# hartikainen/mujoco_mpc

Measured on AMD Instinct MI355X. Metric: candidate rollouts/s (horizon x samples), higher is better.
Workload: dtype f64

## Files before the change

### mujoco_mpc_amd/csrc/host.h

```cpp
#pragma once
#include <stdlib.h>
#include <stdint.h>
#include <string.h>
#include <map>
#include <mutex>
#include <string>
#include <vector>
#include "../../include/mjpc_hip.h"
#include "model.h"

struct PackedModel {
  std::vector<int> ib;
  std::vector<double> db;
  DevModel M;
  Lay L;
  size_t task_i0, task_d0, task_i_cap, task_d_cap;
  size_t cache_i, cache_d;
  size_t hot_i = 0, hot_d = 0;
  int slab_doubles = 0;
  std::string error;
};

namespace mjpc_host {

// ... 87 lines not shown
        case TBL_CONST:
          if (ty < 1 || id < 0 || id > t->num_dbl - ty) return fail(trm + ": constants dbl_data[" + std::to_string(id) + " .. +" + std::to_string(ty) + ") out of range (num_dbl = " + std::to_string(t->num_dbl) + ")");
          len = ty; break;
        case TBL_PARAM: len = t->num_parameter; break;
        case TBL_QPOS: len = M.nq; break;
        case TBL_QVEL: len = M.nv; break;
        case TBL_ACT: if (M.na == 0) return fail(trm + ": ACT on a model without activation states (na = 0)"); len = M.na; break;
        case TBL_CTRL: case TBL_ACTUATOR_FORCE: len = M.nu; break;
        case TBL_KEY_QPOS: if (!obj(M.nkey, "key")) return false; len = M.nq; break;
        case TBL_MOCAP_POS: case TBL_MOCAP_QUAT: case TBL_MOCAP_MAT:
          if (!obj(M.nmocap, "mocap body")) return false;
          len = kind == TBL_MOCAP_POS ? 3 : (kind == TBL_MOCAP_QUAT ? 4 : 9); break;
        case TBL_SUBTREE_COM: case TBL_SUBTREE_LINVEL: if (!obj(M.nbody, "body")) return false; len = 3; break;
        case TBL_POS: case TBL_QUAT: case TBL_MAT: case TBL_XAXIS: case TBL_YAXIS: case TBL_ZAXIS: case TBL_LINVEL: case TBL_ANGVEL:
          if (ty == MJPC_OBJ_BODY || ty == MJPC_OBJ_XBODY) { if (!obj(M.nbody, "body")) return false; }
          else if (ty == MJPC_OBJ_GEOM) { if (!obj(M.ngeom, "geom")) return false; }
          else if (ty == MJPC_OBJ_SITE) { if (!obj(M.nsite, "site")) return false; }
          else return fail(trm + ": unknown object type " + std::to_string(ty));
          len = kind == TBL_QUAT ? 4 : (kind == TBL_MAT ? 9 : 3); break;
        default: return fail(trm + ": unknown source kind " + std::to_string(kind));
      }
      if (op == TBL_OP_SUBQUAT && ((kind != TBL_QUAT && kind != TBL_MOCAP_QUAT) || off != 0)) return fail(trm + ": SUBQUAT takes two quaternion sources (QUAT / MOCAP_QUAT) at offset 0");
      if (off < 0 || off > len - ncomp) return fail(trm + ": components [" + std::to_string(off) + ", " + std::to_string(off) + " + " + std::to_string(ncomp) + ") beyond the source's length " + std::to_string(len));
    }
    row += dim; term += n;
  }
  if (row != t->num_residual) return fail("the blocks end at row " + std::to_string(row) + ", num_residual is " + std::to_string(t->num_residual));
  if (term != nt) return fail("the blocks use " + std::to_string(term) + " of the " + std::to_string(nt) + " terms");
  return true;
}

static inline void make_layout(const PackedModel &p, Lay &L, const MjpcHipModel *m, const MjpcHipTask *t, int P_max, size_t cache_d, size_t cache_i, bool lean = false, bool reg_solver = false, unsigned spill = 0, int *slab_doubles = nullptr, int *scratch = nullptr) {
  const DevModel &M = p.M;
  int nb = m->nbody, nj = m->njnt, nv = m->nv, ng = m->ngeom, ns = m->nsite, nu = m->nu;
  int o = 0, so = 0;
  int nvp = M.nvp, ne = M.nefcmax, nc = M.nconmax, nr = t->num_residual;
#define A_(f, n) L.f = o; o += (int)(n)
#define S_(bit, f, n) if (spill & (bit)) { L.f = LAY_SLAB(so); so += (int)(n); } else { A_(f, n); }
  A_(qpos, m->nq); A_(qvel, nv); A_(ctrl, nu + 1 + 2 * m->na);
  A_(qacc, nv); A_(qacc_ws, nv); A_(qacc_smooth, nv); A_(qfrc_smooth, nv);
  A_(qfrc_bias, nv); A_(qfrc_constraint, nv); A_(actuator_force, nu + 1); A_(mocap_pos, 3 * m->nmocap + 3); A_(mocap_quat, 4 * m->nmocap + 4);
  A_(xpos, 3 * nb); A_(xquat, 4 * nb); A_(xmat, 9 * nb); A_(xipos, 3 * nb); A_(ximat, 9 * nb); A_(xanchor, 3 * nj + 3); A_(xaxis, 3 * nj + 3);
  A_(geom_xpos, 3 * ng + 3); A_(geom_xmat, 9 * ng + 9); A_(site_xpos, 3 * ns + 3);
#define B_(f, n) if (!lean) { A_(f, n); }
  A_(subtree_com, 3 * nb); B_(cinert, 10 * nb); B_(crb, 10 * nb); A_(cdof, 6 * nv + 18); A_(cvel, 6 * nb); B_(cdof_dot, 6 * nv + 18);
  B_(cacc, 6 * nb); B_(cfrc, 6 * nb); B_(cfrc_sub, 6 * nb); A_(subtree_linvel, 3 * nb); A_(bodytmp, 3 * nb);
#undef B_
  A_(qM, nv * nvp + 1); A_(qL, nv * nvp + 1);
  A_(qH, (lean && reg_solver && nv > 32) ? 1 : nv * nvp + 1);
  A_(Linv, nv + 1); A_(Hinv, nv + 1);
  int ja_rows = ((ne - M.nfric + 7) & ~7) + (m->cone == MJPC_CONE_ELLIPTIC ? ((nc + 3) & ~3) : 0) + 4 + ((M.ntfric + 3) & ~3);
  
  S_(SPILL_EFC_J, efc_J, (ne - M.nfric) * nvp + 1);
  int ja_need = 64 + ne * 7 + nc * 17 + (m->cone == MJPC_CONE_ELLIPTIC ? (nc * nv + 7) / 8 + (nc * nv + 3) / 4 + (MJPC_SIDE_JOB > 0 ? 3 : 2) * nv * nvp : 0);
  int ja_size = reg_solver ? ja_need + 1 : ja_rows * nvp + 1;
  if (ja_size < ja_need) ja_size = ja_need;
  S_(SPILL_EFC_JA, efc_JA, ja_size);
  if (scratch) *scratch = ((spill & SPILL_EFC_J) != 0) == ((spill & SPILL_EFC_JA) != 0) ? (ne - M.nfric) * nvp + 1 + ja_size : (ne - M.nfric) * nvp + 1;
  if (lean) {
    int q = L.efc_JA;
    L.cinert = q; q += 10 * nb; L.crb = q; q += 10 * nb; L.cdof_dot = q; q += 6 * nv + 18;
    L.cacc = q; q += 6 * nb; L.cfrc = q; q += 6 * nb; L.cfrc_sub = q; q += 6 * nb;
    if (q > o) o = q;
  }
  S_(SPILL_EFC_VEC, efc_D, ne); S_(SPILL_EFC_VEC, efc_R, ne); S_(SPILL_EFC_VEC, efc_aref, ne); S_(SPILL_EFC_VEC, efc_force, ne);
  S_(SPILL_EFC_VEC, efc_jar, ne); S_(SPILL_EFC_VEC, efc_jv, ne); S_(SPILL_EFC_VEC, efc_floss, ne); S_(SPILL_EFC_VEC, efc_pos, ne);
  L.efc_margin = L.efc_jv; L.efc_diag = L.efc_force;
  S_(SPILL_CONTACT, contact, nc * M.con_stride + 1);
  A_(Ma, nv + 1); A_(grad, nv + 1); A_(Mgrad, nv + 1); A_(search, nv + 1); A_(Mv, nv + 1); A_(vtmp, nv + 1); A_(sgl, 4 * nv + 1);
  if (lean) { L.knot_times = 0; L.knot_values = 0; } else { A_(knot_times, P_max); A_(knot_values, P_max * nu + 1); }
  A_(residual, nr + 1); A_(terms, t->num_term + 1); A_(red, 8); A_(prof, 26);
  A_(scr_a, nv + 1); A_(scr_b, nv + 1);
  if (lean) L.xfrc = 0; else { A_(xfrc, 6 * nb); }
  if (m->noslip_iterations > 0) { S_(SPILL_NOSLIP, noslip, ne * nvp + nc * 36 + 2 * ne + 1); } else L.noslip = 0;
  A_(mc_d, cache_d + 1); A_(mc_i, (cache_i + 2) / 2);
  L.ints = o;
#undef S_
#undef A_
  if (slab_doubles) *slab_doubles = so ? so + nvp + 64 : 0;
  int io = 0;
  L.i_efc_type = io; io += ne; L.i_efc_id = io; io += ne; L.i_efc_state = io; io += ne; L.i_efc_dof = io; io += ne;
  L.i_con = io; io += nc * CONI_STRIDE; L.i_active = io; io += (ne + nc + M.ntfric > MAX_ACTIVE_PAIRS ? ne + nc + M.ntfric : MAX_ACTIVE_PAIRS); L.i_misc = io; io += MISC_INTS;
  L.i_hpair = io; if (!lean) io += M.nhpair + nv;
  L.total_doubles = o + (io + 1) / 2;
}

static inline bool build(PackedModel &p, const MjpcHipModel *m, const MjpcHipTask *t, int P_max, bool use_cache = true, bool lean = false, bool hot_only = false, bool reg_solver = false, int spill_mode = SPILL_NONE) {
  p.ib.clear(); p.db.clear(); p.error.clear(); p.slab_doubles = 0;
  DevModel &M = p.M;
  memset(&M, 0, sizeof(M));
  int nb = m->nbody, nj = m->njnt, nv = m->nv, ng = m->ngeom, ns = m->nsite, nu = m->nu;
  if (nv > 64) { p.error = "nv > 64 not supported (dof bitmask)"; return false; }
  {
    int cnt = 0;
    for (int i = 0; i < nu && m->actuator_dyntype; i++) if (m->actuator_dyntype[i] != MJPC_DYN_NONE) {
      int dt = m->actuator_dyntype[i], a = m->actuator_actadr ? m->actuator_actadr[i] : -1;
      if (dt < 0 || dt > MJPC_DYN_FILTEREXACT) { p.error = "actuator " + std::to_string(i) + ": dyntype " + std::to_string(dt) + " not supported (integrator / filter / filterexact only)"; return false; }
      if (a < 0 || a >= m->na || !m->actuator_dynprm || !m->actuator_actlimited || !m->actuator_actrange) { p.error = "actuator " + std::to_string(i) + ": activation address outside [0, na) or missing actuator_dynprm / actlimited / actrange"; return false; }
      cnt++;
    }
    if (cnt != m->na) { p.error = "na = " + std::to_string(m->na) + " but " + std::to_string(cnt) + " stateful actuators (one activation each)"; return false; } }
  if (m->solver != MJPC_SOL_NEWTON) { p.error = "only the Newton solver (mjSOL_NEWTON) is implemented"; return false; }
  if (m->integrator != MJPC_INT_EULER && m->integrator != MJPC_INT_IMPLICITFAST && m->integrator != MJPC_INT_IMPLICIT) { p.error = "only the Euler (with implicit joint damping), implicitfast and implicit integrators are implemented (not RK4)"; return false; }
  if (m->noslip_iterations < 0) { p.error = "noslip_iterations < 0"; return false; }
  for (int e = 0; e < m->neq; e++) {
    if (!m->eq_type || !m->eq_obj1id || !m->eq_obj2id || !m->eq_active0 || !m->eq_data || !m->eq_solref || !m->eq_solimp) { p.error = "neq > 0 but the eq_* tables are missing"; return false; }
    if (!m->eq_active0[e]) continue;
// ... 466 lines not shown
```

### mujoco_mpc_amd/csrc/linalg.h

```cpp
#pragma once
#include <type_traits>
#include "dmath.h"
#include "model.h"

struct Ctx;

#ifndef MJPC_EMU
DEV double readlane_d(double v, int lane) {
  int lo = __builtin_amdgcn_readlane(__double2loint(v), lane);
  int hi = __builtin_amdgcn_readlane(__double2hiint(v), lane);
  return __hiloint2double(hi, lo);
}
#endif

DEV void chol_factor_lds(double *A, double *Linv, double *tmp, int n, int nvp) {
  for (int j = 0; j < n; j++) {
    SYNC();
    PFOR(ii, n - j) {
      int i = j + ii;
      double s = A[i * nvp + j];
#pragma unroll 4
      for (int k = 0; k < j; k++) s -= A[i * nvp + k] * A[j * nvp + k];
      tmp[i] = s;
    }
    SYNC();
    double t = tmp[j];
    if (t < D_MINVAL) t = D_MINVAL;
    double dj = sqrt(t), inv = 1.0 / dj;
    PFOR(ii, n - j) {
      int i = j + ii;
      A[i * nvp + j] = (i == j) ? dj : tmp[i] * inv;
    }
    if (LANE == 0) Linv[j] = inv;
  }
  SYNC();
}
DEV void chol_solve_lds(const double *L, const double *Linv, double *x, int n, int nvp) {
  for (int i = 0; i < n; i++) {
    SYNC();
    double xi = x[i] * Linv[i];
    SYNC();
    PFOR(kk, n - i - 1) { int k = i + 1 + kk; x[k] -= L[k * nvp + i] * xi; }
    if (LANE == 0) x[i] = xi;
  }
  for (int i = n - 1; i >= 0; i--) {
    SYNC();
    double xi = x[i] * Linv[i];
    SYNC();
    PFOR(k, i) x[k] -= L[i * nvp + k] * xi;
    if (LANE == 0) x[i] = xi;
  }
  SYNC();
}

#ifndef MJPC_EMU
template <int N>
struct LDLRegs { double lo[N], up[N], rinv; };
struct LDLExtra { const double *x[3]; int n; const double *row; };

template <int I, int E, class F>
DEV void static_for(F &&f) {
  if constexpr (I < E) { f(std::integral_constant<int, I>{}); static_for<I + 1, E>(f); }
}
template <int N>
DEV void ldl_load_row(const double *A, int nvp, const LDLExtra *ex, double *a, double &dg) {
  const int i = LANE;
  const bool act = i < N;
  if (ex && ex->row) {
    double d0 = 1.0;
    static_for<0, N>([&](auto jc) { constexpr int j = decltype(jc)::value; a[j] = act ? ex->row[j] : 0.0; d0 = (j == i) ? ex->row[j] : d0; });
    dg = act ? d0 : 1.0;
  } else {
    static_for<0, N>([&](auto jc) { constexpr int j = decltype(jc)::value; a[j] = act ? A[(j <= i) ? i * nvp + j : j * nvp + i] : 0.0; });
    dg = act ? A[i * nvp + i] : 1.0;
  }
  if (ex && ex->n > 0) {
    const int nx = ex->n;
    double t[3][N], td[3];
#pragma unroll
    for (int w = 0; w < 3; w++) {
      const double *X = ex->x[w < nx ? w : 0];
      static_for<0, N>([&](auto jc) { constexpr int j = decltype(jc)::value; t[w][j] = X[(j <= i && act) ? i * nvp + j : (act ? j * nvp + i : 0)]; });
      td[w] = X[act ? i * nvp + i : 0];
      if (w + 1 >= nx) break;
    }
    __builtin_amdgcn_sched_barrier(0);
#pragma unroll
    for (int w = 0; w < 3; w++) {
      if (w >= nx) break;
      static_for<0, N>([&](auto jc) { constexpr int j = decltype(jc)::value; a[j] += act ? t[w][j] : 0.0; });
      dg += act ? td[w] : 0.0;
    }
  }
}
template <int N>
DEV void ldl_factor_regs(const double *A, int nvp, LDLRegs<N> &f, const LDLExtra *ex = nullptr) {
  static_assert(N >= 1 && N <= 64, "one matrix row per lane");
  const int i = LANE;
  const bool act = i < N;
  double a[N];
  double dg;
  ldl_load_row<N>(A, nvp, ex, a, dg);
  static_for<1, N>([&](auto kc) {
    constexpr int k = N - decltype(kc)::value;
    double rk = readlane_d(fast_rcp(dg < D_MINVAL ? D_MINVAL : dg), k);
    double hk = a[k];
    double l = (i < k) ? hk * rk : 0.0;
    dg -= l * hk;
    static_for<0, (k + 7) / 8>([&](auto gc) {
      constexpr int j0 = decltype(gc)::value * 8;
      double sj[8];
      static_for<0, 8>([&](auto qc) { constexpr int q = decltype(qc)::value; if constexpr (j0 + q < k) sj[q] = readlane_d(a[j0 + q], k); });
      __builtin_amdgcn_sched_barrier(0);
      static_for<0, 8>([&](auto qc) { constexpr int q = decltype(qc)::value; if constexpr (j0 + q < k) a[j0 + q] -= l * sj[q]; });
      __builtin_amdgcn_sched_barrier(0);
    });
    f.up[k] = l;
  });
  f.up[0] = 0.0;
  if (dg < D_MINVAL) dg = D_MINVAL;
  f.rinv = fast_rcp(dg);
  static_for<0, N>([&](auto jc) { constexpr int j = decltype(jc)::value; f.lo[j] = (act && j < i) ? a[j] * f.rinv : 0.0; });
}
template <int N>
DEV double ldl_solve_regs(const LDLRegs<N> &f, double xi) {
  static_for<1, N>([&](auto kc) { constexpr int k = N - decltype(kc)::value; xi -= f.up[k] * readlane_d(xi, k); });
  xi *= f.rinv;
  static_for<0, N - 1>([&](auto jc) { constexpr int j = decltype(jc)::value; xi -= f.lo[j] * readlane_d(xi, j); });
  return xi;
}
template <int N> constexpr int tree_depth(int k) { int d = 0; for (int a = DofTree<N>::parent(k); a >= 0; a = DofTree<N>::parent(a)) d++; return d; }
template <int N> constexpr int tree_nth_anc(int k, int n) { int a = DofTree<N>::parent(k); for (int q = 0; q < n; q++) a = DofTree<N>::parent(a); return a; }
template <int N> constexpr int tree_height(int k) {
  int h = 0;
  for (int c = k + 1; c < N; c++) if (DofTree<N>::parent(c) == k) { int hc = tree_height<N>(c) + 1; if (hc > h) h = hc; }
  return h;
}
template <int N> constexpr int tree_nlevel() { int h = 0; for (int k = 0; k < N; k++) { int hk = tree_height<N>(k); if (hk > h) h = hk; } return h + 1; }
template <int N> constexpr int tree_level_npair(int H) { int n = 0; for (int k = N - 1; k >= 1; k--) if (tree_height<N>(k) == H) n += tree_depth<N>(k); return n; }
template <int N> constexpr int tree_level_pair(int H, int e, bool pivot) {
  for (int k = N - 1; k >= 1; k--) if (tree_height<N>(k) == H) {
    int d = tree_depth<N>(k);
    if (e < d) return pivot ? k : tree_nth_anc<N>(k, e);
    e -= d;
  }
// ... 150 lines not shown
```

### mujoco_mpc_amd/csrc/model.h

```cpp
#pragma once
#include <stdint.h>

#define CON_STRIDE_ELLIPTIC 45
#define NVP_OF(n) ((((n) + 1)) | 1)
#define CON_STRIDE_PLAIN 27
#define CON_DIST 0
#define CON_POS 1
#define CON_FRAME 4
#define CON_INCLUDEMARGIN 13
#define CON_FRICTION 14
#define CON_SOLREF 19
#define CON_SOLIMP 21
#define CON_MU 26
#define CON_H 27
#ifndef MJPC_SIDE_JOB
#define MJPC_SIDE_JOB 0
#endif
#define CONI_STRIDE 4
#define MAX_ACTIVE_PAIRS 192
#define EFC_CON_ID(ci, dim, r0) ((ci) | ((dim) << 8) | ((r0) << 16))
#define EFC_CON_CI(id) ((id) & 255)
#define EFC_CON_DIM(id) (((id) >> 8) & 255)
#define EFC_CON_R0(id) ((id) >> 16)

template <int N> struct DofTree { static constexpr bool known = false; static constexpr int parent(int) { return -1; } static constexpr int real_parent(int) { return -1; } };
template <> struct DofTree<18> {
  static constexpr bool known = true;
  static constexpr int parent(int k) { constexpr int p[18] = {-1, 0, 1, 2, 3, 4, 5, 6, 7, 5, 9, 10, 5, 12, 13, 5, 15, 16}; return p[k]; }
  static constexpr int real_parent(int k) { return parent(k); }
};
template <> struct DofTree<27> {
  static constexpr bool known = true;
  static constexpr int parent(int k) {
    constexpr int p[27] = {-1, 0, 1, 2, 3, 4, 5, 6, 7, 8, 9, 10, 11, 12, 13, 8, 15, 16, 17, 18, 19, 5, 21, 22, 5, 24, 25};
    return p[k];
  }
  static constexpr int real_parent(int k) { return parent(k); }
};
template <> struct DofTree<33> {
  static constexpr bool known = true;
  static constexpr int parent(int k) {
    constexpr int p[33] = {-1, 0, 1, -1, 3, 4, 5, 6, 7,  8, 9, 10, 11, 12, 13, 10, 15, 16, 17, 10, 19, 20, 21, 10, 23, 24, 25, 26, 10, 28, 29, 30, 31};
    return p[k];
  }
  static constexpr int real_parent(int k) { return k == 9 ? -1 : parent(k); }
};
template <int N> constexpr bool dof_tree_matches(const int *dof_parentid) {
  if (!DofTree<N>::known) return false;
  for (int k = 0; k < N; k++) if (dof_parentid[k] != DofTree<N>::real_parent(k)) return false;
  return true;
}
static inline int pattern_parent(int nv, int tree_ok, const int *dof_parentid, int k) {
  if (!tree_ok) return dof_parentid[k];
  if (nv == 18) return DofTree<18>::parent(k);
  if (nv == 27) return DofTree<27>::parent(k);
  if (nv == 33) return DofTree<33>::parent(k);
  return dof_parentid[k];
// ... 137 lines not shown
```

### mujoco_mpc_amd/csrc/solver_reg.h

```cpp
#pragma once
#ifndef MJPC_EMU
#ifndef LS_PREDICT
#define LS_PREDICT 1
#endif

template <int NVT> struct HLay {
  static constexpr int G0 = 64 / NVT;
  static constexpr int G = G0 < 1 ? 1 : (G0 > NVT ? NVT : G0);
  static constexpr int CB = (NVT + G - 1) / G;
};
DEV int readlane_i(int v, int lane) { return __builtin_amdgcn_readlane(v, lane); }
#define LSR_STRIDE 7
#define LSC_STRIDE 17
#define LS_ROWREC(c) ((c).efc_JA + 64)
#define LS_CONREC(c) ((c).efc_JA + 64 + (c).M->nefcmax * LSR_STRIDE)

template <int NVT>
DEV void hblock_add_rows(const Ctx &c, double *h, unsigned long long mask, int rbase, double wlane, int hi, int j0) {
  constexpr int nvp = NVP_OF(NVT), CB = HLay<NVT>::CB;
  while (mask) {
    int b0 = (int)__builtin_ctzll(mask); mask &= mask - 1;
    int b1 = b0; double sel1 = 0.0;
    if (mask) { b1 = (int)__builtin_ctzll(mask); mask &= mask - 1; sel1 = 1.0; }
    double w0 = readlane_d(wlane, b0), w1 = readlane_d(wlane, b1) * sel1;
// ... 30 lines not shown
  const int nefc = c.nefc, ns = c.nsingle;
  for (int base = 0; base < nefc; base += NLANE) {
    int r = base + LANE, rc = r < nefc ? r : nefc - 1;
    int st = c.efc_state[rc], type = c.efc_type[rc];
    double D = c.efc_D[rc];
    int flag = r < nefc && r >= ns && st == STATE_QUADRATIC;
    (void)type;
    unsigned long long mask = __builtin_amdgcn_ballot_w64(flag != 0);
    hblock_add_rows<NVT>(c, hq, mask, base, D, hi, j0);
  }
}

template <int NVT>
DEV void newton_grad_reg(Ctx &c, int hi, int hg, bool hact) {
  constexpr int nvp = NVP_OF(NVT), G = HLay<NVT>::G;
  const int ns = c.nsingle, n = c.nefc - ns;
  double part = 0;
  const int trips = (n + G - 1) / G;
  for (int t0 = 0; t0 < trips; t0 += 8) {
    double f[8], j[8];
#pragma unroll
    for (int u = 0; u < 8; u++) {
      int rr = (t0 + u) * G + hg;
      int r = ns + (rr < n ? rr : 0);
      f[u] = c.efc_force[r]; j[u] = c.efc_J[r * nvp + hi];
    }
    __builtin_amdgcn_sched_barrier(0);
#pragma unroll
    for (int u = 0; u < 8; u++) { int rr = (t0 + u) * G + hg; double pr = j[u] * f[u]; part += (rr < n) ? pr : 0.0; }
    __builtin_amdgcn_sched_barrier(0);
  }
  double *sc = c.efc_JA;
  if (hact) sc[hg * NVT + hi] = part;
  SYNC();
  if (LANE < NVT) {
    int i = LANE;
    double jtf = 0;
#pragma unroll
    for (int g = 0; g < G; g++) jtf += sc[g * NVT + i];
    double gr = c.Ma[i] - c.qfrc_smooth[i] - (c.sgl[i] + c.sgl[2 * NVT + i]) - jtf;
    c.grad[i] = gr;
    c.Mgrad[i] = gr;
  }
  SYNC();
}

#define HX_JOBW 18
#define HX_SIDEFROM 21
#define HX_NITEMS 45
#define HX_WDONE HX_HDONE
#define JOBW(seq, np, kind) (((seq) << 4) | ((np) << 2) | (kind))
#define MJPC_NW (MJPC_NH + 1)
#define CONE_BASE(c) ((c).efc_JA + 64 + (c).M->nefcmax * LSR_STRIDE + (c).M->nconmax * LSC_STRIDE)
#define CONE_DOFS(c) ((unsigned char *)CONE_BASE(c))
#define CONE_ITEMS(c) ((unsigned short *)(CONE_BASE(c) + ((c).M->nconmax * NVT + 7) / 8))
#define CONE_PARTIAL(c, w) (CONE_BASE(c) + ((c).M->nconmax * NVT + 7) / 8 + ((c).M->nconmax * NVT + 3) / 4 + (w) * (NVT * NVP_OF(NVT)))

template <int NVT, int DIMT>
DEV void cone_rows(const Ctx &c, double *part, int p0, int pstep) {
  constexpr int nvp = NVP_OF(NVT);
  const int nitems = uniform_i(c.misc[HX_NITEMS]), stride = c.M->con_stride;
  const unsigned short *items = CONE_ITEMS(c);
  const double *crec = LS_CONREC(c);
  for (int it0 = p0 * NLANE; it0 < nitems; it0 += pstep * NLANE) {
    const int it = it0 + LANE;
    const bool valid = it < nitems;
    const int item = items[valid ? it : 0];
    const int ci = item & 255, a = item >> 8;
    const int info = ((const int *)(crec + ci * LSC_STRIDE + 14))[0];
    const int r0 = info >> 16, dim = (info >> 8) & 255;
    const unsigned char *dofs = CONE_DOFS(c) + ci * NVT;
    const int i = dofs[a];
    const int st = c.efc_state[r0];
    const double *cf = c.contact + ci * stride + CON_H;
    double P[DIMT], Q[DIMT], T[DIMT], ji[DIMT];
#pragma unroll
    for (int k = 0; k < DIMT; k++) { P[k] = cf[k]; Q[k] = cf[6 + k]; T[k] = cf[12 + k]; }
    const double *Jr = c.efc_J + r0 * nvp;
#pragma unroll
    for (int k = 0; k < DIMT; k++) ji[k] = Jr[(DIMT <= 3 || k < dim ? k : 0) * nvp + i];
    __builtin_amdgcn_sched_barrier(0);
    const bool active = valid && st == STATE_CONE;
#if defined(MJPC_PROFILE) && !defined(MJPC_EMU)
    if (MJPC_PROFILE_WAVE != 0 && WAVE_ID() == MJPC_PROFILE_WAVE) { int na_ = __builtin_popcountll(__builtin_amdgcn_ballot_w64(active)); if (LANE == 0) { c.prof[23] += na_; c.prof[22] += (it0 == p0 * NLANE); } }
#endif
    if constexpr (DIMT > 3) {
#pragma unroll
      for (int k = 3; k < DIMT; k++) { const bool in = k < dim; P[k] = in ? P[k] : 0.0; Q[k] = in ? Q[k] : 0.0; T[k] = in ? T[k] : 0.0; ji[k] = in ? ji[k] : 0.0; }
    }
    double pi = P[0] * ji[0], qi = Q[1] * ji[1];
#pragma unroll
    for (int k = 1; k < DIMT; k++) { pi += P[k] * ji[k]; if (k > 1) qi += Q[k] * ji[k]; }
    double t[DIMT];
    t[0] = P[0] * pi + Q[0] * ji[0];
#pragma unroll
    for (int k = 1; k < DIMT; k++) t[k] = P[k] * pi - Q[k] * qi + (T[k] * T[k]) * ji[k];
    double *prow = part + i * nvp;
    PROFW(c, 16);
    for (int b = 0; __builtin_amdgcn_ballot_w64(active && b <= a) != 0; b += 2) {
      const bool on0 = active && b <= a, on1 = active && b + 1 <= a;
      const int j0 = dofs[on0 ? b : 0], j1 = dofs[on1 ? b + 1 : 0];
      double x0[DIMT], x1[DIMT];
#pragma unroll
      for (int k = 0; k < DIMT; k++) { x0[k] = Jr[(DIMT <= 3 || k < dim ? k : 0) * nvp + j0]; x1[k] = Jr[(DIMT <= 3 || k < dim ? k : 0) * nvp + j1]; }
      __builtin_amdgcn_sched_barrier(0);
      double v0 = t[0] * x0[0], v1 = t[0] * x1[0];
#pragma unroll
      for (int k = 1; k < DIMT; k++) { v0 += t[k] * x0[k]; v1 += t[k] * x1[k]; }
      if (on0) __builtin_amdgcn_ds_atomic_fadd_f64((__attribute__((address_space(3))) double *)(prow + j0), v0);
      if (on1) __builtin_amdgcn_ds_atomic_fadd_f64((__attribute__((address_space(3))) double *)(prow + j1), v1);
    }
  }
}

#if MJPC_HELPER
DEV int jobw_load(const Ctx &c) { return __builtin_amdgcn_readfirstlane(__hip_atomic_load(c.misc + HX_JOBW, __ATOMIC_RELAXED, __HIP_MEMORY_SCOPE_WORKGROUP)); }
template <int NVT>
DEV int job_post(Ctx &c, int kind, int &side_in) {
  if (c.M->cone != 1) return 0;
  const int seq = ++c.hseq;
  if (MJPC_SIDE_JOB > 0 && !side_in && (seq & 255) >= MJPC_SIDE_JOB) {
    const int base = seq & ~255;
    int ok = 0;
    for (int n = 0; n < (1 << 21); n++) {
      int from = __builtin_amdgcn_readfirstlane(__hip_atomic_load(c.misc + HX_SIDEFROM, __ATOMIC_RELAXED, __HIP_MEMORY_SCOPE_WORKGROUP));
      if (from > base) { ok = 1; break; }
    }
    if (!ok) c.warning |= WARN_SYNC;
    side_in = 1;
  }
  const int np = MJPC_NH + (side_in ? 1 : 0);
  flag_set(c.misc + HX_JOBW, JOBW(seq, np, kind));
  return np;
}
DEV void job_wait(Ctx &c, int np) {
  const int seq = c.hseq;
  for (int k = 0; k < np; k++) if (!flag_wait(c.misc + HX_WDONE + k, seq)) c.warning |= WARN_SYNC;
}
template <int NVT, int DIMT>
DEV void worker_job(Ctx &c, int W, int np, int seq) {
  constexpr int nvp = NVP_OF(NVT);
  PROFW(c, 12);
  double *part = CONE_PARTIAL(c, W);
  PFOR(e, NVT * nvp) part[e] = 0;
  PROFW(c, 15);
  cone_rows<NVT, DIMT>(c, part, W, np);
  PROFW(c, 13);
  flag_set(c.misc + HX_WDONE + W, seq);
  PROFW(c, 14);
}
template <int NVT, int DIMT>
DEV void worker_loop_d(Ctx &c, int W, int last) {
  if (W != 0 && c.nefc > 0 && !flag_wait(c.misc + HX_LSREC, (last >> 8) + 1)) return;
  for (;;) {
    int word = 0, ok = 0;
    for (int n = 0; n < (1 << 21); n++) { word = jobw_load(c); if ((word >> 4) > last) { ok = 1; break; } }
    __builtin_amdgcn_fence(__ATOMIC_ACQUIRE, "workgroup");
    if (!ok) return;
    const int kind = word & 3, np = (word >> 2) & 3;
    if (kind == 0) return;
    last = word >> 4;
    if (W < np) worker_job<NVT, DIMT>(c, W, np, last);
  }
}
template <int NVT>
DEV void worker_loop(Ctx &c, int W, int last) {
  if (c.M->cone != 1) return;
  if (c.M->maxdim <= 3) worker_loop_d<NVT, 3>(c, W, last); else worker_loop_d<NVT, 6>(c, W, last);
}
template <int NVT>
DEV void side_worker(Ctx &c, int t) {
  if (c.M->cone != 1 || MJPC_SIDE_JOB <= 0) return;
  const int base = t * 256;
  int word = jobw_load(c);
  int last = base;
  if ((word >> 4) > base) {
    if ((word & 3) == 0) return;
    last = word >> 4;
  }
  if (LANE == 0) __hip_atomic_store(c.misc + HX_SIDEFROM, last + 1, __ATOMIC_RELAXED, __HIP_MEMORY_SCOPE_WORKGROUP);
  worker_loop<NVT>(c, MJPC_NH, last);
}
#endif

template <int NVT, int DIMT>
DEV void newton_assemble(Ctx &c, const double *hq, int hi, int hg, int j0, bool hact) {
  constexpr int nvp = NVP_OF(NVT), CB = HLay<NVT>::CB;
  double a[CB];
  const double dg = c.sgl[NVT + hi] + c.sgl[3 * NVT + hi];
#pragma unroll
  for (int q = 0; q < CB; q++) a[q] = hq[q] + ((j0 + q == hi) ? dg : 0.0);
#if !MJPC_HELPER
  if (c.M->cone == 1) {
    double *part = CONE_PARTIAL(c, 0);
    PFOR(e, NVT * nvp) part[e] = 0;
    cone_rows<NVT, DIMT>(c, part, 0, 1);
    SYNC();
#pragma unroll
    for (int q = 0; q < CB; q++) a[q] += (hact && j0 + q <= hi) ? part[hi * nvp + j0 + q] : 0.0;
  }
#endif
  if (hact) {
#pragma unroll
    for (int q = 0; q < CB; q++) if (j0 + q < NVT) c.qH[hi * nvp + j0 + q] = a[q];
  }
  SYNC();
}
template <int NVT>
DEV void newton_direction_np(Ctx &c, int np) {
  if (np > 0) {
    LDLExtra ex;
    ex.row = nullptr;
    ex.n = np;
#pragma unroll
    for (int w = 0; w < 3; w++) ex.x[w] = CONE_PARTIAL(c, w < np ? w : 0);
    newton_direction_sum<NVT>(c, ex);
  } else newton_direction<NVT>(c);
}

template <int NVT>
DEV void newton_direction_rows(Ctx &c, const double *hq, int hi, bool hact, int np) {
  if constexpr (HLay<NVT>::G != 1) return;
  double row[NVT];
  const double dg = c.sgl[NVT + hi] + c.sgl[3 * NVT + hi];
#pragma unroll
  for (int q = 0; q < NVT; q++) row[q] = hact ? hq[q] + ((q == hi) ? dg : 0.0) : 0.0;
  LDLExtra ex;
  ex.row = row;
  ex.n = np;
#pragma unroll
  for (int w = 0; w < 3; w++) ex.x[w] = CONE_PARTIAL(c, w < np ? w : 0);
  chol_factor_solve_reg<NVT>(c.qH, c.Mgrad, NVP_OF(NVT), c.M->tree_ok && !c.cross, &ex);
  PROF(c, 17);
}

template <int DIMT>
struct LSReg {
  double lo[LS_RPL], hi[LS_RPL], hD[LS_RPL], F[LS_RPL], X[LS_RPL], V[LS_RPL], DV[LS_RPL], DVV[LS_RPL], rJ[LS_RPL];
  int rinfo[LS_RPL];
  double N0[LS_CPL], NV[LS_CPL], t0[LS_CPL], t1[LS_CPL], t2[LS_CPL], c0[LS_CPL], c1[LS_CPL], c2[LS_CPL], mu[LS_CPL], Dm[LS_CPL];
  int on[LS_CPL], cdim[LS_CPL], crow[LS_CPL], cwasq[LS_CPL];
  int nslot, ncslot;
};

template <int NVT>
DEV void ls_records_build(Ctx &c) {
  constexpr int nvp = NVP_OF(NVT);
  const int nefc = c.nefc, ncon = c.ncon, ns = c.nsingle, nfr = c.M->nfric;
  double *rrec = LS_ROWREC(c), *crec = LS_CONREC(c);
  PFOR(r, nefc) {
    int type = c.efc_type[r], dof = c.efc_dof[r];
    double D = c.efc_D[r], f = c.efc_floss[r], Rf = c.efc_R[r] * f;
    int single = r < ns;
    double rj = single ? (r < nfr ? 1.0 : c.efc_J[r * nvp + dof]) : 0.0;
    int quad = type != CNSTR_CONTACT_ELLIPTIC;
    int fric = quad && type <= CNSTR_FRICTION_TENDON;
    double *o = rrec + r * LSR_STRIDE;
    o[0] = fric ? -Rf : (quad ? -1e300 : -1.0); o[1] = fric ? Rf : (quad ? 0.0 : 1.0);
    o[2] = quad ? 0.5 * D : 0.0; o[3] = fric ? f : 0.0; o[4] = rj;
    ((int *)(o + 5))[0] = quad | (fric << 1) | ((quad && single) << 2) | ((single ? dof : 0) << 8);
    o[6] = D;
  }
  int nc_lane = 0;
  PFOR(ci, ncon) {
    int dim = c.con_i[ci * CONI_STRIDE], i = c.con_i[ci * CONI_STRIDE + 3];
    const double *cc = c.contact + ci * c.M->con_stride;
    int on = dim > 1 && c.efc_type[i] == CNSTR_CONTACT_ELLIPTIC;
    double mu = cc[CON_MU];
    double *o = crec + ci * LSC_STRIDE;
    for (int j = 0; j < 6; j++) {
      int use = on && j < dim;
      double fr = j == 0 ? mu : cc[CON_FRICTION + j - 1];
      double Dj = c.efc_D[use ? i + j : i];
      o[j] = use ? Dj * fast_rcp(fr * fr) : 0.0;
      o[6 + j] = use ? fr : 0.0;
    }
    o[12] = on ? mu : 0.0;
    o[13] = on ? c.efc_D[i] * fast_rcp(mu * mu * (1 + mu * mu)) : 0.0;
    ((int *)(o + 14))[0] = on | (dim << 8) | (i << 16);
    int nc = 0;
    if (on) {
      unsigned long long m = MDM()[MI(geom_bodyid)[c.con_i[ci * CONI_STRIDE + 1]]] | MDM()[MI(geom_bodyid)[c.con_i[ci * CONI_STRIDE + 2]]];
      unsigned char *dl = CONE_DOFS(c) + ci * NVT;
      while (m) { int dd = (int)__builtin_ctzll(m); m &= m - 1; dl[nc++] = (unsigned char)dd; }
    }
    ((int *)(o + 14))[2] = nc;
    nc_lane = nc;
  }
  {
    int total, off = wave_excl_scan(nc_lane, &total);
    unsigned short *il = CONE_ITEMS(c) + off;
    for (int a = 0; a < nc_lane; a++) il[a] = (unsigned short)(LANE | (a << 8));
    if (LANE == 0) c.misc[HX_NITEMS] = total;
  }
  SYNC();
}

template <int NVT, int DIMT>
DEV void ls_load_reg(Ctx &c, LSReg<DIMT> &d) {
  const int nefc = c.nefc, ncon = c.ncon, last = c.nefc - 1;
  const double *rrec = LS_ROWREC(c), *crec = LS_CONREC(c);
  d.nslot = (nefc + NLANE - 1) / NLANE; d.ncslot = (ncon + NLANE - 1) / NLANE;
#pragma unroll
  for (int k = 0; k < LS_RPL; k++) {
    d.lo[k] = -1; d.hi[k] = 1; d.hD[k] = 0; d.F[k] = 0; d.X[k] = 0; d.V[k] = 0; d.DV[k] = 0; d.DVV[k] = 0; d.rJ[k] = 0; d.rinfo[k] = 0;
    if (k < d.nslot) {
      int r = LANE + NLANE * k, rc = r < nefc ? r : last;
      const double *o = rrec + rc * LSR_STRIDE;
      double lo = o[0], hi = o[1], hD = o[2], F = o[3], rj = o[4];
      int info = ((const int *)(o + 5))[0], st = c.efc_state[rc];
      double v = c.efc_jv[rc], x = c.efc_jar[rc];
      __builtin_amdgcn_sched_barrier(0);
      const bool ok = r < nefc;
      d.X[k] = ok ? x : 0.0; d.V[k] = ok ? v : 0.0;
      d.lo[k] = ok ? lo : -1.0; d.hi[k] = ok ? hi : 1.0; d.hD[k] = ok ? hD : 0.0; d.F[k] = ok ? F : 0.0; d.rJ[k] = rj;
      d.rinfo[k] = ok ? (info | ((st == STATE_QUADRATIC) << 3)) : 0;
      double dv = 2 * d.hD[k] * d.V[k];
      d.DV[k] = dv; d.DVV[k] = dv * d.V[k];
    }
  }
#pragma unroll
  for (int q = 0; q < LS_CPL; q++) {
    d.on[q] = 0; d.mu[q] = 0; d.Dm[q] = 0; d.cdim[q] = 0; d.crow[q] = 0; d.cwasq[q] = 0;
    d.N0[q] = 0; d.NV[q] = 0; d.t0[q] = 0; d.t1[q] = 0; d.t2[q] = 0; d.c0[q] = 0; d.c1[q] = 0; d.c2[q] = 0;
    if (q < d.ncslot) {
      int ci = LANE + NLANE * q, cic = ci < ncon ? ci : ncon - 1;
      const double *o = crec + cic * LSC_STRIDE;
      int info = ((const int *)(o + 14))[0];
      double E[DIMT], fr[DIMT];
#pragma unroll
      for (int j = 0; j < DIMT; j++) { E[j] = o[j]; fr[j] = o[6 + j]; }
      double mu = o[12], Dm = o[13];
      int on = (ci < ncon) && (info & 1), dim = (info >> 8) & 255, i = info >> 16;
      double jv[DIMT], jr[DIMT];
#pragma unroll
      for (int j = 0; j < DIMT; j++) { int rj = i + j < nefc ? i + j : last; jv[j] = c.efc_jv[rj]; jr[j] = c.efc_jar[rj]; }
      int st0 = c.efc_state[i];
      __builtin_amdgcn_sched_barrier(0);
      d.on[q] = on; d.mu[q] = on ? mu : 0.0; d.Dm[q] = on ? Dm : 0.0; d.cdim[q] = dim; d.crow[q] = i;
      d.cwasq[q] = st0 == STATE_QUADRATIC;
      double t0 = 0, t1 = 0, t2 = 0, c0 = 0, c1 = 0, c2 = 0, n0 = 0, nv_ = 0;
#pragma unroll
      for (int j = 0; j < DIMT; j++) {
        double u = jr[j] * fr[j], v = jv[j] * fr[j], eu = E[j] * u, ev = E[j] * v;
        c0 += 0.5 * eu * u; c1 += eu * v; c2 += 0.5 * ev * v;
        if (j == 0) { n0 = u; nv_ = v; } else { t0 += u * u; t1 += u * v; t2 += v * v; }
// ... 318 lines not shown
```

Measured before the change: 25890.

## Compute cone Hessian per matrix entry instead of per-contact row scatter with atomics

Replaces the per-contact, per-dof row scatter into per-worker partial Hessian matrices, which used LDS atomic adds, with a per-entry formulation. Each lower-triangular entry (i,j) gets a bitmask of the contacts whose support covers both dofs, and a lane sums their contributions directly. Entries with many contacts are split across four lanes and reduced with shuffles. Worker partials now write disjoint entries of a single shared matrix, so the LDL load reads one extra matrix instead of up to three, and the zeroing of each per-worker partial is removed. The trade-off is a per-step mask-building pass over all entries and contacts in ls_records_build, plus a changed scratch layout.

```diff
diff --git a/mujoco_mpc_amd/csrc/host.h b/mujoco_mpc_amd/csrc/host.h
--- a/mujoco_mpc_amd/csrc/host.h
+++ b/mujoco_mpc_amd/csrc/host.h
@@ -163,7 +163,10 @@
   int ja_rows = ((ne - M.nfric + 7) & ~7) + (m->cone == MJPC_CONE_ELLIPTIC ? ((nc + 3) & ~3) : 0) + 4 + ((M.ntfric + 3) & ~3);
   
   S_(SPILL_EFC_J, efc_J, (ne - M.nfric) * nvp + 1);
-  int ja_need = 64 + ne * 7 + nc * 17 + (m->cone == MJPC_CONE_ELLIPTIC ? (nc * nv + 7) / 8 + (nc * nv + 3) / 4 + (MJPC_SIDE_JOB > 0 ? 3 : 2) * nv * nvp : 0);
+  const int nitem = CONE_NITEM(nv);
+  const int cone_now = nitem + (nitem + 3) / 4 + nv * nvp;
+  const int cone_was = (nc * nv + 7) / 8 + (nc * nv + 3) / 4 + (MJPC_SIDE_JOB > 0 ? 3 : 2) * nv * nvp;
+  int ja_need = 64 + ne * 7 + nc * 17 + (m->cone == MJPC_CONE_ELLIPTIC ? (cone_now > cone_was ? cone_now : cone_was) : 0);
   int ja_size = reg_solver ? ja_need + 1 : ja_rows * nvp + 1;
   if (ja_size < ja_need) ja_size = ja_need;
   S_(SPILL_EFC_JA, efc_JA, ja_size);
diff --git a/mujoco_mpc_amd/csrc/linalg.h b/mujoco_mpc_amd/csrc/linalg.h
--- a/mujoco_mpc_amd/csrc/linalg.h
+++ b/mujoco_mpc_amd/csrc/linalg.h
@@ -56,7 +56,7 @@
 #ifndef MJPC_EMU
 template <int N>
 struct LDLRegs { double lo[N], up[N], rinv; };
-struct LDLExtra { const double *x[3]; int n; const double *row; };
+struct LDLExtra { const double *x; const double *row; };
 
 template <int I, int E, class F>
 DEV void static_for(F &&f) {
@@ -74,23 +74,14 @@
     static_for<0, N>([&](auto jc) { constexpr int j = decltype(jc)::value; a[j] = act ? A[(j <= i) ? i * nvp + j : j * nvp + i] : 0.0; });
     dg = act ? A[i * nvp + i] : 1.0;
   }
-  if (ex && ex->n > 0) {
-    const int nx = ex->n;
-    double t[3][N], td[3];
-#pragma unroll
-    for (int w = 0; w < 3; w++) {
-      const double *X = ex->x[w < nx ? w : 0];
-      static_for<0, N>([&](auto jc) { constexpr int j = decltype(jc)::value; t[w][j] = X[(j <= i && act) ? i * nvp + j : (act ? j * nvp + i : 0)]; });
-      td[w] = X[act ? i * nvp + i : 0];
-      if (w + 1 >= nx) break;
-    }
+  if (ex && ex->x) {
+    const double *X = ex->x;
+    double t[N], td;
+    static_for<0, N>([&](auto jc) { constexpr int j = decltype(jc)::value; t[j] = X[(j <= i && act) ? i * nvp + j : (act ? j * nvp + i : 0)]; });
+    td = X[act ? i * nvp + i : 0];
     __builtin_amdgcn_sched_barrier(0);
-#pragma unroll
-    for (int w = 0; w < 3; w++) {
-      if (w >= nx) break;
-      static_for<0, N>([&](auto jc) { constexpr int j = decltype(jc)::value; a[j] += act ? t[w][j] : 0.0; });
-      dg += act ? td[w] : 0.0;
-    }
+    static_for<0, N>([&](auto jc) { constexpr int j = decltype(jc)::value; a[j] += act ? t[j] : 0.0; });
+    dg += act ? td : 0.0;
   }
 }
 template <int N>
diff --git a/mujoco_mpc_amd/csrc/model.h b/mujoco_mpc_amd/csrc/model.h
--- a/mujoco_mpc_amd/csrc/model.h
+++ b/mujoco_mpc_amd/csrc/model.h
@@ -3,6 +3,11 @@
 
 #define CON_STRIDE_ELLIPTIC 45
 #define NVP_OF(n) ((((n) + 1)) | 1)
+#define CONE_HEAVY 4
+#define CONE_NENT(nv) ((nv) * ((nv) + 1) / 2)
+#define CONE_ROOM(nv) (((nv) * NVP_OF(nv) - CONE_NENT(nv) - (CONE_NENT(nv) + 3) / 4) * 4 / 5)
+#define CONE_EXTRA(nv) ((CONE_ROOM(nv) < 0 ? 0 : (CONE_ROOM(nv) > 96 ? 96 : CONE_ROOM(nv))) / 3 * 3)
+#define CONE_NITEM(nv) (CONE_NENT(nv) + CONE_EXTRA(nv))
 #define CON_STRIDE_PLAIN 27
 #define CON_DIST 0
 #define CON_POS 1
diff --git a/mujoco_mpc_amd/csrc/solver_reg.h b/mujoco_mpc_amd/csrc/solver_reg.h
--- a/mujoco_mpc_amd/csrc/solver_reg.h
+++ b/mujoco_mpc_amd/csrc/solver_reg.h
@@ -106,64 +106,65 @@
 #define JOBW(seq, np, kind) (((seq) << 4) | ((np) << 2) | (kind))
 #define MJPC_NW (MJPC_NH + 1)
 #define CONE_BASE(c) ((c).efc_JA + 64 + (c).M->nefcmax * LSR_STRIDE + (c).M->nconmax * LSC_STRIDE)
-#define CONE_DOFS(c) ((unsigned char *)CONE_BASE(c))
-#define CONE_ITEMS(c) ((unsigned short *)(CONE_BASE(c) + ((c).M->nconmax * NVT + 7) / 8))
-#define CONE_PARTIAL(c, w) (CONE_BASE(c) + ((c).M->nconmax * NVT + 7) / 8 + ((c).M->nconmax * NVT + 3) / 4 + (w) * (NVT * NVP_OF(NVT)))
+#define CONE_MASKS(c) ((unsigned long long *)CONE_BASE(c))
+#define CONE_ENTS(c) ((unsigned short *)(CONE_BASE(c) + CONE_NITEM(NVT)))
+#define CONE_MAT(c) (CONE_BASE(c) + CONE_NITEM(NVT) + (CONE_NITEM(NVT) + 3) / 4)
 
 template <int NVT, int DIMT>
-DEV void cone_rows(const Ctx &c, double *part, int p0, int pstep) {
+DEV void cone_entries(Ctx &c, int W, int np) {
   constexpr int nvp = NVP_OF(NVT);
-  const int nitems = uniform_i(c.misc[HX_NITEMS]), stride = c.M->con_stride;
-  const unsigned short *items = CONE_ITEMS(c);
+  const int nitem = uniform_i(c.misc[HX_NITEMS]), stride = c.M->con_stride, ncon = c.ncon;
+  const unsigned short *ents = CONE_ENTS(c);
+  const unsigned long long *masks = CONE_MASKS(c);
   const double *crec = LS_CONREC(c);
-  for (int it0 = p0 * NLANE; it0 < nitems; it0 += pstep * NLANE) {
-    const int it = it0 + LANE;
-    const bool valid = it < nitems;
-    const int item = items[valid ? it : 0];
-    const int ci = item & 255, a = item >> 8;
-    const int info = ((const int *)(crec + ci * LSC_STRIDE + 14))[0];
-    const int r0 = info >> 16, dim = (info >> 8) & 255;
-    const unsigned char *dofs = CONE_DOFS(c) + ci * NVT;
-    const int i = dofs[a];
-    const int st = c.efc_state[r0];
-    const double *cf = c.contact + ci * stride + CON_H;
-    double P[DIMT], Q[DIMT], T[DIMT], ji[DIMT];
-#pragma unroll
-    for (int k = 0; k < DIMT; k++) { P[k] = cf[k]; Q[k] = cf[6 + k]; T[k] = cf[12 + k]; }
-    const double *Jr = c.efc_J + r0 * nvp;
-#pragma unroll
-    for (int k = 0; k < DIMT; k++) ji[k] = Jr[(DIMT <= 3 || k < dim ? k : 0) * nvp + i];
-    __builtin_amdgcn_sched_barrier(0);
-    const bool active = valid && st == STATE_CONE;
+  double *cm = CONE_MAT(c);
+  unsigned long long conemask;
+  {
+    const bool has = LANE < ncon;
+    const int info = ((const int *)(crec + (has ? LANE : 0) * LSC_STRIDE + 14))[0];
+    const int st = c.efc_state[has ? info >> 16 : 0];
+    conemask = __builtin_amdgcn_ballot_w64(has && (info & 1) && st == STATE_CONE);
+  }
 #if defined(MJPC_PROFILE) && !defined(MJPC_EMU)
-    if (MJPC_PROFILE_WAVE != 0 && WAVE_ID() == MJPC_PROFILE_WAVE) { int na_ = __builtin_popcountll(__builtin_amdgcn_ballot_w64(active)); if (LANE == 0) { c.prof[23] += na_; c.prof[22] += (it0 == p0 * NLANE); } }
-#endif
-    if constexpr (DIMT > 3) {
-#pragma unroll
-      for (int k = 3; k < DIMT; k++) { const bool in = k < dim; P[k] = in ? P[k] : 0.0; Q[k] = in ? Q[k] : 0.0; T[k] = in ? T[k] : 0.0; ji[k] = in ? ji[k] : 0.0; }
-    }
-    double pi = P[0] * ji[0], qi = Q[1] * ji[1];
-#pragma unroll
-    for (int k = 1; k < DIMT; k++) { pi += P[k] * ji[k]; if (k > 1) qi += Q[k] * ji[k]; }
-    double t[DIMT];
-    t[0] = P[0] * pi + Q[0] * ji[0];
-#pragma unroll
-    for (int k = 1; k < DIMT; k++) t[k] = P[k] * pi - Q[k] * qi + (T[k] * T[k]) * ji[k];
-    double *prow = part + i * nvp;
-    PROFW(c, 16);
-    for (int b = 0; __builtin_amdgcn_ballot_w64(active && b <= a) != 0; b += 2) {
-      const bool on0 = active && b <= a, on1 = active && b + 1 <= a;
-      const int j0 = dofs[on0 ? b : 0], j1 = dofs[on1 ? b + 1 : 0];
-      double x0[DIMT], x1[DIMT];
-#pragma unroll
-      for (int k = 0; k < DIMT; k++) { x0[k] = Jr[(DIMT <= 3 || k < dim ? k : 0) * nvp + j0]; x1[k] = Jr[(DIMT <= 3 || k < dim ? k : 0) * nvp + j1]; }
+  if (MJPC_PROFILE_WAVE != 0 && WAVE_ID() == MJPC_PROFILE_WAVE && LANE == 0) { c.prof[23] += __builtin_popcountll(conemask); c.prof[22] += 1; }
+#endif
+  PROFW(c, 15);
+  const int ngroup = (nitem + 3) >> 2;
+  for (int g0 = W; g0 < ngroup; g0 += np * (NLANE / 4)) {
+    const int q = (g0 + np * (LANE >> 2)) * 4 + (LANE & 3);
+    const bool valid = q < nitem;
+    const int ent = ents[valid ? q : 0];
+    const int i = ent & 63, j = (ent >> 8) & 63;
+    const bool split = valid && (ent >> 15) != 0;
+    unsigned long long m = valid ? masks[valid ? q : 0] & conemask : 0ull;
+    double sum = 0;
+    while (m) {
+      const int ci = (int)__builtin_ctzll(m); m &= m - 1;
+      const int info = ((const int *)(crec + ci * LSC_STRIDE + 14))[0];
+      const int r0 = info >> 16, dim = (info >> 8) & 255;
+      const double *cf = c.contact + ci * stride + CON_H;
+      double P[DIMT], Q[DIMT], T[DIMT], ji[DIMT], x[DIMT];
+#pragma unroll
+      for (int k = 0; k < DIMT; k++) { P[k] = cf[k]; Q[k] = cf[6 + k]; T[k] = cf[12 + k]; }
+      const double *Jr = c.efc_J + r0 * nvp;
+#pragma unroll
+      for (int k = 0; k < DIMT; k++) { const int kk = (DIMT <= 3 || k < dim ? k : 0) * nvp; ji[k] = Jr[kk + i]; x[k] = Jr[kk + j]; }
       __builtin_amdgcn_sched_barrier(0);
-      double v0 = t[0] * x0[0], v1 = t[0] * x1[0];
-#pragma unroll
-      for (int k = 1; k < DIMT; k++) { v0 += t[k] * x0[k]; v1 += t[k] * x1[k]; }
-      if (on0) __builtin_amdgcn_ds_atomic_fadd_f64((__attribute__((address_space(3))) double *)(prow + j0), v0);
-      if (on1) __builtin_amdgcn_ds_atomic_fadd_f64((__attribute__((address_space(3))) double *)(prow + j1), v1);
-    }
+      double pi = P[0] * ji[0], qi = Q[1] * ji[1];
+#pragma unroll
+      for (int k = 1; k < DIMT; k++) { pi += P[k] * ji[k]; if (k > 1) qi += Q[k] * ji[k]; }
+      double t[DIMT];
+      t[0] = P[0] * pi + Q[0] * ji[0];
+#pragma unroll
+      for (int k = 1; k < DIMT; k++) t[k] = P[k] * pi - Q[k] * qi + (T[k] * T[k]) * ji[k];
+      double v = t[0] * x[0];
+#pragma unroll
+      for (int k = 1; k < DIMT; k++) v += t[k] * x[k];
+      sum += v;
+    }
+    const double s1 = __shfl_down(sum, 1, 4), s2 = __shfl_down(sum, 2, 4), s3 = __shfl_down(sum, 3, 4);
+    const double whole = split ? ((sum + s1) + s2) + s3 : sum;
+    if (valid && (!split || (LANE & 3) == 0)) cm[i * nvp + j] = whole;
   }
 }
 
@@ -193,12 +194,8 @@
 }
 template <int NVT, int DIMT>
 DEV void worker_job(Ctx &c, int W, int np, int seq) {
-  constexpr int nvp = NVP_OF(NVT);
   PROFW(c, 12);
-  double *part = CONE_PARTIAL(c, W);
-  PFOR(e, NVT * nvp) part[e] = 0;
-  PROFW(c, 15);
-  cone_rows<NVT, DIMT>(c, part, W, np);
+  cone_entries<NVT, DIMT>(c, W, np);
   PROFW(c, 13);
   flag_set(c.misc + HX_WDONE + W, seq);
   PROFW(c, 14);
@@ -246,9 +243,8 @@
   for (int q = 0; q < CB; q++) a[q] = hq[q] + ((j0 + q == hi) ? dg : 0.0);
 #if !MJPC_HELPER
   if (c.M->cone == 1) {
-    double *part = CONE_PARTIAL(c, 0);
-    PFOR(e, NVT * nvp) part[e] = 0;
-    cone_rows<NVT, DIMT>(c, part, 0, 1);
+    const double *part = CONE_MAT(c);
+    cone_entries<NVT, DIMT>(c, 0, 1);
     SYNC();
 #pragma unroll
     for (int q = 0; q < CB; q++) a[q] += (hact && j0 + q <= hi) ? part[hi * nvp + j0 + q] : 0.0;
@@ -265,9 +261,7 @@
   if (np > 0) {
     LDLExtra ex;
     ex.row = nullptr;
-    ex.n = np;
-#pragma unroll
-    for (int w = 0; w < 3; w++) ex.x[w] = CONE_PARTIAL(c, w < np ? w : 0);
+    ex.x = CONE_MAT(c);
     newton_direction_sum<NVT>(c, ex);
   } else newton_direction<NVT>(c);
 }
@@ -281,9 +275,7 @@
   for (int q = 0; q < NVT; q++) row[q] = hact ? hq[q] + ((q == hi) ? dg : 0.0) : 0.0;
   LDLExtra ex;
   ex.row = row;
-  ex.n = np;
-#pragma unroll
-  for (int w = 0; w < 3; w++) ex.x[w] = CONE_PARTIAL(c, w < np ? w : 0);
+  ex.x = np > 0 ? CONE_MAT(c) : nullptr;
   chol_factor_solve_reg<NVT>(c.qH, c.Mgrad, NVP_OF(NVT), c.M->tree_ok && !c.cross, &ex);
   PROF(c, 17);
 }
@@ -315,7 +307,7 @@
     ((int *)(o + 5))[0] = quad | (fric << 1) | ((quad && single) << 2) | ((single ? dof : 0) << 8);
     o[6] = D;
   }
-  int nc_lane = 0;
+  unsigned long long supp = 0;
   PFOR(ci, ncon) {
     int dim = c.con_i[ci * CONI_STRIDE], i = c.con_i[ci * CONI_STRIDE + 3];
     const double *cc = c.contact + ci * c.M->con_stride;
@@ -332,20 +324,64 @@
     o[12] = on ? mu : 0.0;
     o[13] = on ? c.efc_D[i] * fast_rcp(mu * mu * (1 + mu * mu)) : 0.0;
     ((int *)(o + 14))[0] = on | (dim << 8) | (i << 16);
-    int nc = 0;
-    if (on) {
-      unsigned long long m = MDM()[MI(geom_bodyid)[c.con_i[ci * CONI_STRIDE + 1]]] | MDM()[MI(geom_bodyid)[c.con_i[ci * CONI_STRIDE + 2]]];
-      unsigned char *dl = CONE_DOFS(c) + ci * NVT;
-      while (m) { int dd = (int)__builtin_ctzll(m); m &= m - 1; dl[nc++] = (unsigned char)dd; }
-    }
-    ((int *)(o + 14))[2] = nc;
-    nc_lane = nc;
-  }
-  {
-    int total, off = wave_excl_scan(nc_lane, &total);
-    unsigned short *il = CONE_ITEMS(c) + off;
-    for (int a = 0; a < nc_lane; a++) il[a] = (unsigned short)(LANE | (a << 8));
-    if (LANE == 0) c.misc[HX_NITEMS] = total;
+    if (on && c.M->con_stride > CON_H) { double *ch = c.contact + ci * c.M->con_stride + CON_H; for (int j = dim; j < 6; j++) { ch[j] = 0; ch[6 + j] = 0; ch[12 + j] = 0; } }
+    if (on) supp = MDM()[MI(geom_bodyid)[c.con_i[ci * CONI_STRIDE + 1]]] | MDM()[MI(geom_bodyid)[c.con_i[ci * CONI_STRIDE + 2]]];
+  }
+  if (c.M->cone == 1) {
+    constexpr int NE = CONE_NENT(NVT), NPASS = (NE + NLANE - 1) / NLANE;
+    double *cm = CONE_MAT(c);
+    PFOR(e, NVT * nvp) cm[e] = 0;
+    unsigned long long *masks = CONE_MASKS(c);
+    unsigned short *ents = CONE_ENTS(c);
+    const int slo = (int)(unsigned)supp, shi = (int)(unsigned)(supp >> 32);
+    unsigned long long emask[NPASS];
+    int eij[NPASS];
+#pragma unroll
+    for (int ps = 0; ps < NPASS; ps++) {
+      const int e = ps * NLANE + LANE;
+      int i = (int)((sqrtf(8.0f * (float)e + 1.0f) - 1.0f) * 0.5f);
+      while ((i + 1) * (i + 2) / 2 <= e) i++;
+      while (i * (i + 1) / 2 > e) i--;
+      const int j = e - i * (i + 1) / 2;
+      const unsigned long long need = (1ull << (i & 63)) | (1ull << j);
+      unsigned long long mask = 0;
+      for (int cc = 0; cc < ncon; cc++) {
+        const unsigned long long s = ((unsigned long long)(unsigned)readlane_i(shi, cc) << 32) | (unsigned)readlane_i(slo, cc);
+        mask |= ((s & need) == need) ? (1ull << cc) : 0ull;
+      }
+      emask[ps] = e < NE ? mask : 0ull;
+      eij[ps] = (i & 63) | (j << 8);
+    }
+    int nitem = 0, nsplit = 0;
+#pragma unroll
+    for (int ps = 0; ps < NPASS; ps++) {
+      const unsigned long long mask = emask[ps];
+      int total, off = wave_flag_scan(__builtin_popcountll(mask) > CONE_HEAVY, &total);
+      const bool take = __builtin_popcountll(mask) > CONE_HEAVY && nsplit + off < CONE_EXTRA(NVT) / 3;
+      if (take) {
+        unsigned long long part[4] = {0, 0, 0, 0};
+        int rank = 0;
+        for (unsigned long long m2 = mask; m2; m2 &= m2 - 1, rank++) {
+          const unsigned long long bit = m2 & (0 - m2);
+#pragma unroll
+          for (int p_ = 0; p_ < 4; p_++) part[p_] |= (rank & 3) == p_ ? bit : 0ull;
+        }
+        const int at = (nsplit + off) * 4;
+#pragma unroll
+        for (int p_ = 0; p_ < 4; p_++) { masks[at + p_] = part[p_]; ents[at + p_] = (unsigned short)(eij[ps] | 0x8000); }
+        emask[ps] = 0;
+      }
+      nsplit += total < CONE_EXTRA(NVT) / 3 - nsplit ? total : CONE_EXTRA(NVT) / 3 - nsplit;
+    }
+    nitem = nsplit * 4;
+#pragma unroll
+    for (int ps = 0; ps < NPASS; ps++) {
+      const unsigned long long mask = emask[ps];
+      int total, off = wave_flag_scan(mask != 0, &total);
+      if (mask) { masks[nitem + off] = mask; ents[nitem + off] = (unsigned short)eij[ps]; }
+      nitem += total;
+    }
+    if (LANE == 0) c.misc[HX_NITEMS] = nitem;
   }
   SYNC();
 }
```

After: 25850. About the same (-0.1%).
